# fuxiao0719/PanopticNeRF

Measured on AMD Instinct MI355X. Metric: Msamples/sec (coarse+fine), KITTI-360 1408x376, higher is better.
Workload: dtype bf16

## Files before the change

### panopticnerf_amd/csrc/asm/gen_mlp_tt.py

```python
#!/usr/bin/env python3
import struct
import sys
from contextlib import contextmanager

V_T2 = 15
NSLOT, SLOT = 4, 33 * 1024
P = 4
D, SKIP = 8, 4

V_TID, V_LANE16, V_FRAG, V_BIAS, V_T0, V_DMA, V_LB4, V_TRACE = 0, 1, 2, 6, 10, 11, 14, 15
V_T1 = 1
V_RING, V_ACC = 16, 32
V_EX, V_ED = 160, 192
V_G = 208
V_ZZ, V_ZN, V_DN, V_LW = 240, 242, 244, 246
V_IN = 224
V_TMP = 208
V_PTMP = 248
V_AUXA = V_PTMP + 6
V_LWA = V_IN + 2
A0, A1 = 0, 128
S_IMG, S_RAYS, S_Z, S_S, S_N, S_MAGIC, S_SHIFT, S_NGRP, S_NWG, S_REC, S_RECF, S_PS, S_NSEM, S_NINST, S_CLK = 4, 6, 8, 10, 11, 12, 13, 14, 15, 16, 18, 20, 22, 23, 24
S_WAVE, S_W4K, S_GRP, S_PIECE, S_T0, S_T1 = 26, 27, 28, 30, 34, 35
S_VALID, S_LAST = 36, 40
# ... 32 lines not shown
    def __init__(self, kind, base):
        self.kind, self.base = kind, base

    def reg(self, i, n=1):
        return (ar if self.kind == "a" else vr)(self.base + i, n)


class Sim:
    def __init__(self, name, cap):
        self.name, self.cap, self.q, self.n = name, cap, [], 0

    def push(self, certain=True):
        self.n += 1
        self.q.append((self.n, certain))
        return self.n

    def wait_count(self, tag):
        if tag is None or not any(t == tag for t, _ in self.q):
            return None
        idx = [t for t, _ in self.q].index(tag)
        n = sum(1 for _, c in self.q[idx + 1:] if c)
        n = min(n, self.cap)
        self.q = self.q[idx + 1:]
        return n

    def drain(self):
        self.q = []

    def state(self):
        return [c for _, c in self.q]


class Gen:
    def __init__(self, nbs, nbi, name, trace=False, abl=0, depth=2, softmax=False, tap=0):
        self.depth = depth
        self.tap = tap
        self.softmax = softmax
        self.nbs, self.nbi, self.name, self.trace, self.abl = nbs, nbi, name, trace, abl
        self.nstamp = 0
        self.o = []
        self.nlabel = 0
        self.lgkm = Sim("lgkm", 15)
        self.vm = Sim("vm", 63)
        self.side, self.side_lo, self.outbox, self.capture = [], [], [], None
        self.ring_tags = [None] * P
        self.piece_tag = {}
        self.pending_pack = None
        self.g2_acc = self.park_acc = None
        self.m0 = None
        self.logit_units = []
        self.acc_free = list(range(8))
        self.lwr_acc = self.lwr_tag = None
        self.aux_tags = {}
        self.build_plan()
        self.build_units()
        self.stream = []
        for u in self.units:
            u["frag0"] = len(self.stream)
            self.stream += [(sl, of) for sl, of, _, _ in self.unit_frags(u)]

    def build_plan(self):
        L = []

        def add(name, nblk, segs, fbc, mode):
            nks = sum(n for _, n in segs)
            if fbc * nks + 1 > 33:
                fbc = 1
            L.append(dict(name=name, nblk=nblk, segs=segs, nks=nks, fbc=fbc, mode=mode))
        for i in range(D):
            if i == 0:
                add("L0", 8, [("ex", 4)], 8, "relu")
            elif i - 1 == SKIP:
                add("L%d" % i, 8, [("ex", 4), ("h", 16)], 2, "relu")
            else:
                add("L%d" % i, 8, [("h", 16)], 2, "relu")
        add("feature", 8, [("h", 16)], 2, "linear")
        add("views", 4, [("F", 16), ("ed", 2)], 2, "relu")
        add("rgbs", 1, [("g", 8), ("hh", 16)], 1, "rgbs")
        if self.depth == 1:
            if self.nbs:
                add("sem1", self.nbs, [("tap", 16)], self.nbs, "logits")
            if self.nbi:
                add("inst1", 1, [("tap", 16)], 1, "logits")
        else:
            if self.nbs:
                add("sem0", 4, [("tap", 16)], 2, "relu")
            if self.nbi:
                add("inst0", 4, [("tap", 16)], 2, "relu")
            if self.nbs:
                add("sem1", self.nbs, [("shs", 8)], self.nbs, "logits")
            if self.nbi:
                add("inst1", 1, [("shi", 8)], 1, "logits")
# ... 494 lines not shown
            e("s_lshl_b32 s%d, s%d, 3" % (S_T0, S_GRP))
            e("s_lshl_b32 s%d, s%d, 1" % (S_SAVE, S_WAVE))
            e("s_add_u32 s%d, s%d, s%d" % (S_T0, S_T0, S_SAVE))
            e("s_add_u32 s%d, s%d, %d" % (S_T0, S_T0, t))
            e("s_mul_i32 s%d, s%d, s%d" % (S_SAVE, S_T0, S_RECF))
            e("s_mul_hi_i32 s%d, s%d, s%d" % (S_SAVE + 1, S_T0, S_RECF))
            e("s_lshl_b64 s[%d:%d], s[%d:%d], 2" % (S_SAVE, S_SAVE + 1, S_SAVE, S_SAVE + 1))
            e("s_add_u32 s%d, s%d, s%d" % (S_REC_T + 2 * t, S_REC, S_SAVE))
            e("s_addc_u32 s%d, s%d, s%d" % (S_REC_T + 2 * t + 1, S_REC + 1, S_SAVE + 1))
            e("s_lshl_b32 s%d, s%d, 2" % (S_SAVE, S_NSEM))
            e("s_add_u32 s%d, s%d, s%d" % (S_REC_I + 2 * t, S_REC_T + 2 * t, S_SAVE))
            e("s_addc_u32 s%d, s%d, 0" % (S_REC_I + 2 * t + 1, S_REC_T + 2 * t + 1))
            e("s_lshl_b32 s%d, s%d, 5" % (S_T0, S_T0))
            e("v_and_b32 v%d, 31, v%d" % (d, V_TID))
            e("v_or_b32 v%d, s%d, v%d" % (d, S_T0, d))
            e("v_lshlrev_b32 v%d, 4, v%d" % (d, d))
            e("v_mov_b32 v%d, v%d" % (T[4], V_LW + t))
            e("v_mov_b32 v%d, v%d" % (T[5], acc + 0))
            e("v_mov_b32 v%d, v%d" % (T[6], acc + 1))
            e("v_mov_b32 v%d, v%d" % (T[7], acc + 2))
            e("s_and_b64 s[%d:%d], s[%d:%d], s[%d:%d]" % (S_SAVE, S_SAVE + 1, VAL, VAL + 1, S_HI0, S_HI0 + 1))
            e("s_mov_b64 exec, s[%d:%d]" % (S_SAVE, S_SAVE + 1))
            self.vm_op("global_store_dwordx4 v%d, %s, s[%d:%d]" % (d, vr(T[4], 4), S_PS, S_PS + 1))
            e("s_mov_b64 exec, 1")
            e("v_mov_b32 v%d, s%d" % (x, S_Q))
            e("v_mov_b32 v%d, 0" % d)
            self.vm_op("global_store_dword v%d, v%d, s[%d:%d]" % (d, x, S_REC_T + 2 * t, S_REC_T + 2 * t + 1))
            e("s_mov_b64 exec, -1")
        self.q(28, stores)

    def acc_reg(self, i):
        return V_ACC + 16 * i

    def acc_take(self, n):
        assert len(self.acc_free) >= n, ("accumulators exhausted", self.acc_free)
        got, self.acc_free = self.acc_free[:n], self.acc_free[n:]
        return got

    def acc_release(self, ids):
        self.acc_free = sorted(set(self.acc_free) | set(ids))

    def arm_plan(self, u):
        c = self.chunks[u["chunk"]]
        l = self.layers[u["layer"]]
        slot = u["chunk"] % NSLOT
        bias_off = c["nfb"] * l["nks"] * 1024
        u["accs"], u["arm_tags"] = {}, []
        plans = []
        for bi, blk in enumerate(u["blocks"]):
            b_in_chunk = blk - c["fb"]
            for t in range(2):
                key = (bi, t)
                ops = []

                def take(key=key):
                    while not self.acc_free and self.side_busy():
                        self.drain_side(8)
                    u["accs"][key] = self.acc_take(1)[0]
                if t == 1:
                    plans.append([take])
                    continue
                if l["mode"] == "logits":
                    def first(key=key, slot=slot, take=take):
                        take()
                        self.e("v_add_u32 v%d, 0x%x, v%d" % (self.acc_reg(u["accs"][key]), slot * SLOT, V_LB4))
                    ops.append(first)
                    for r in list(range(1, 16)) + [0]:
                        ops.append(lambda key=key, r=r, off=bias_off + b_in_chunk * 128: u["arm_tags"].append(
                            self.lds_read("ds_read_b32 v%d, v%d offset:%d" % (self.acc_reg(u["accs"][key]) + r, self.acc_reg(u["accs"][key]), off))))
                else:
                    for m in range(4):
                        def rd(key=key, m=m, off=bias_off + b_in_chunk * 128 + m * 32, take=take):
                            if m == 0:
                                take()
                            a = self.acc_reg(u["accs"][key])
                            u["arm_tags"].append(self.lds_read("ds_read_b128 %s, v%d offset:%d" % (vr(a + 4 * m, 4), V_BIAS + slot, off)))
                        ops.append(rd)
                plans.append(ops)
        return plans

    def pack_ops(self, u):
        l = self.layers[u["layer"]]
        if not self.trace:
            return self.pack_ops_pipelined(u)
        out = []
        for bi, blk in enumerate(u["blocks"]):
            for t in range(2):
                a = self.acc_reg(u["accs"][(bi, t)])
                dst = self.out_block(l, blk, t)
                for p in range(8):
                    def fn(a=a, p=p, dst=dst, relu=(l["mode"] == "relu"), k=len(out)):
# ... 34 lines not shown
                self.e("v_pk_max_i16 v%d, v%d, 0" % (d if kind == "v" else T[k % 3], T[k % 3]))

        def store(k):
            _, kind, d, _ = pairs[k]
            if kind == "a":
                self.e("v_accvgpr_write_b32 a%d, v%d" % (d, T[k % 3]))

        def final_at(k):
            kind = pairs[k][1]
            return k + 2 if kind == "a" else (k + 1 if relu else k)
        out = []
        for j in range(n + 2):
            def fn(j=j):
                if 0 <= j - 2 < n:
                    store(j - 2)
                if 0 <= j - 1 < n:
                    activate(j - 1)
                if j < n:
                    convert(j)
            done = [(pairs[k][1], pairs[k][2]) for k in range(max(0, j - 2), min(n, j + 1)) if final_at(k) == j]
            out.append((done, fn, pairs[min(j, n - 1)][3]))
        return out

    @staticmethod
    def tile_at(ks, t):
        return 1 - t if ks == 0 else t

    def b_operand(self, u, ks, t):
        l = self.layers[u["layer"]]
        seg, k = self.seg_of_ks(l, ks)
        li = u["layer"]
        return self.loc_of(seg, li, t, k)

    def emit_unit(self, ui, side_budget=3):
        U = self.units
        u = U[ui]
        l = self.layers[u["layer"]]
        c = self.chunks[u["chunk"]]
        frags = self.unit_frags(u)
        nm = 2 * len(frags)
        swap = l["mode"] == "logits"
        e = self.e
        e("; ==== unit %d: %s blocks %s (chunk %d, slot %d), %d MFMAs" % (ui, l["name"], u["blocks"], u["chunk"], u["chunk"] % NSLOT, nm))
        self.stamp(ui)
        if l["name"] == "L%d" % (SKIP + 2) and u["blocks"][0] == 0:
            self.queue_inputs_early()
        if l["name"] == "views" and u["blocks"] == [0]:
            self.drain_side()
        if l["name"] == "views" and u["blocks"] == [1]:
            self.park()
        if l["name"] == (("sem0" if self.nbs else "inst0") if self.depth == 2 else "sem1") and u["blocks"][0] == 0:
            self.unpark()
        if l["name"] == "views" and u["blocks"] == [2]:
            self.g2_acc = self.acc_take(1)[0]
        prev = self.pending_pack
        self.pending_pack = None
        packs = prev["ops"] if prev else []
        reads = {}
        for i in range(nm):
            f, t = i // 2, i % 2
            loc = self.b_operand(u, frags[f][2], self.tile_at(frags[f][2], t))
            for r in range(4):
                reads.setdefault((loc.kind, loc.base + r), i)
        nxt = U[ui + 1] if ui + 1 < len(U) else None
        plans = self.arm_plan(nxt) if nxt is not None else []
        musts, dls, pack_fns = [], [], set()
        by_acc = {}
        for dst, fn, a in packs:
            by_acc.setdefault(a, []).append((dst, fn))
        k = 0
        for a, lst in by_acc.items():
            for dst, fn in lst:
                musts.append(fn if not self.abl & 4 else (lambda: None))
                pack_fns.add(musts[-1])
                if isinstance(dst, list):
                    dd = [reads[d] for d in dst if d in reads]
                    dls.append(min(dd) if dd else None)
                else:
                    dls.append(reads.get(dst))
            musts.append(lambda a=a: self.acc_release([a]))
            dls.append(None)
            if k < len(plans):
                for op in plans[k]:
                    musts.append(op)
                    dls.append(None)
                k += 1
        for kk in range(k, len(plans)):
            for op in plans[kk]:
                musts.append(op)
                dls.append(None)
        lwr_from = None
        if nxt is None and (self.logit_units or l["mode"] == "logits"):
            lwr_from = len(musts)
            for op in self.lwr_ops():
                musts.append(op)
                dls.append(None)
        n = len(musts)
        pos = []
        late = not packs and n > 0 and nxt is not None
        for j in range(n):
            spread = 1 + (j * max(1, nm - 6)) // max(1, n) if not late else (2 * nm) // 3 + (j * max(1, nm // 3 - 5)) // max(1, n)
            pos.append(spread if dls[j] is None else min(spread, max(0, dls[j] - 2)))
        if lwr_from is not None:
            nl = n - lwr_from
            for j in range(lwr_from, n):
                pos[j] = max(pos[j], min(nm - 2, nm // 2 + ((j - lwr_from) * max(1, nm // 2 - 3)) // nl))
        for j in range(n - 2, -1, -1):
            pos[j] = min(pos[j], pos[j + 1])
        must_at = {}
        for j, g in enumerate(pos):
            must_at.setdefault(g, []).append(j)
        piece_at = {}
        cu = [k for k, x in enumerate(U) if x["chunk"] == u["chunk"]]
        c3 = (u["chunk"] + 3) % self.NC
        npieces = self.pieces_of(c3)
        k_in = cu.index(ui)
        mine = [j for j in range(npieces) if (j * len(cu)) // npieces == k_in]
        cost = [3 * sum(1 for j in must_at.get(g, []) if j < n and dls[j] is not None or (j < n and musts[j] in pack_fns)) +
                sum(1 for j in must_at.get(g, [])) for g in range(nm)]
        for idx, j in enumerate(mine):
            span = max(len(mine) + 1, nm - 3)
            lo = 1 + (idx * span) // max(1, len(mine))
            hi = max(lo + 1, 1 + ((idx + 1) * span) // max(1, len(mine)))
            g = min(range(lo, min(hi, nm - 1)), key=lambda x: (cost[x], x))
            cost[g] += 2
            piece_at.setdefault(g, []).append(j)
        first_wait_done = False
        for i in range(nm):
            f, t = i // 2, i % 2
            slot, off, ks, bi = frags[f]
            gi = u["frag0"] + f
            if t == 0:
                if not first_wait_done:
                    for tg in u["arm_tags"][-1:]:
                        self.wait_lgkm(tg)
                    first_wait_done = True
                self.wait_lgkm(self.ring_tags[gi % P])
            tile = self.tile_at(ks, t)
            a = self.acc_reg(u["accs"][(bi, tile)])
            c_in = self.acc_reg(u["accs"][(bi, 0)]) if ks == 0 else a
            bloc = self.b_operand(u, ks, tile)
            ring = vr(V_RING + 4 * (gi % P), 4)
            if swap:
                e("v_mfma_f32_32x32x16_bf16 %s, %s, %s, %s" % (vr(a, 16), bloc.reg(0, 4), ring, vr(c_in, 16)))
            else:
                e("v_mfma_f32_32x32x16_bf16 %s, %s, %s, %s" % (vr(a, 16), ring, bloc.reg(0, 4), vr(c_in, 16)))
            if t == 1:
                gn = gi + P - 1
                if gn < len(self.stream):
                    sl, of = self.stream[gn]
                    self.ring_tags[gn % P] = self.lds_read("ds_read_b128 %s, v%d offset:%d" % (vr(V_RING + 4 * (gn % P), 4), V_FRAG + sl, of))
            for j in must_at.get(i, []):
                musts[j]()
            for j in ([] if self.abl & 1 else piece_at.get(i, [])):
                if j == 0:
                    self.chunk_base(c3)
                tg = self.piece(c3, j)
                self.piece_tag[c3] = tg
            self.drain_side(1 if l["name"].startswith("L") or l["name"] in ("feature", "views") else 3 if late else 2)
        for g in sorted(must_at):
            assert g < nm, (g, nm)
        if l["mode"] in ("relu", "linear"):
            self.pending_pack = dict(ops=self.pack_ops(u), accs=list(u["accs"].values()))
        elif l["mode"] == "rgbs":
            for t in range(2):
                self.rgbs_epilogue(t, self.acc_reg(u["accs"][(0, t)]))
            ids = list(u["accs"].values())
            self.q(0, lambda: self.defer(lambda: self.acc_release(ids)))
            self.queue_inputs_late()
            self.acc_release([self.g2_acc])
            self.g2_acc = None
            if not self.nbs:
                self.unpark()
        else:
            self.logit_units.append(u)
        if u["last_of_chunk"]:
            c2 = (u["chunk"] + 2) % self.NC
            if not self.abl & 2:
                self.wait_vm(self.piece_tag.get(c2))
                e("s_barrier")
            d = u["chunk"] + 1
            while d < self.NC and self.chunks[d].get("dummy"):
                e("; ==== dummy chunk %d (slot %d)" % (d, d % NSLOT))
                c3 = (d + 3) % self.NC
# ... 145 lines not shown
            for r in ([] if self.softmax else range(16)):
                for t in ts:
                    for k, (u, bi, blk, inst) in enumerate(blocks):
                        a = self.acc_reg(u["accs"][(bi, t)])
                        if r == 0:
                            e("v_fma_f32 v%d, v%d, v%d, 0" % (sums[t][k], lwr_reg(t, 0), a))
                        else:
                            e("v_fmac_f32 v%d, v%d, v%d" % (sums[t][k], lwr_reg(t, r), a + r))
            for t in ts:
                tags[t] = [self.lds_read("ds_bpermute_b32 v%d, v%d, v%d" % (oth[t][k], adr, sums[t][k])) for k in range(nb)]

        def stores(t):
            for k in range(nb):
                self.wait_lgkm(tags[t][k])
                e("v_add_f32 v%d, v%d, v%d" % (oth[t][k], sums[t][k], oth[t][k]))
            for k, (u, bi, blk, inst) in enumerate(blocks):
                e("s_mov_b64 exec, s[%d:%d]" % (S_MSK + 2 * k, S_MSK + 2 * k + 1))
                base = (S_REC_I if inst else S_REC_T) + 2 * t
                self.vm_op("global_store_dword v%d, v%d, s[%d:%d] offset:%d" % (V_LB4, oth[t][k], base, base + 1, 4 + 128 * blk))
            e("s_mov_b64 exec, -1")
        self.stamp(len(self.units) + 4)
        if self.softmax:
            self.tail_softmax(blocks, lwr_reg, tag_lwr)
        fmas((0, 1))
        self.stamp(len(self.units) + 5)
        stores(0)
        stores(1)
        for u in self.logit_units:
            self.acc_release(list(u["accs"].values()))
        self.acc_release(self.lwr_acc)
        self.lwr_acc = None
        self.logit_units = []

    def queue_inputs_early(self):
        def which():
            with self.atomic():
                self.e("s_add_u32 s%d, s%d, s%d" % (S_GRP2, S_GRP, S_NWG))
                self.e("s_cmp_lt_i32 s%d, s%d" % (S_GRP2, S_NGRP))
                self.e("s_cselect_b32 s%d, s%d, s%d" % (S_GRP2, S_GRP2, S_GRP))
        self.q(3, which)
        tags = {}
        for t in range(2):
            self.q(34, (lambda t=t: tags.__setitem__(t, self.fetch_tile(t, S_GRP2))))
        for t in range(2):
            self.q(1, (lambda t=t: self.wait_vm(tags[t])))
            for cost, fn in self.encode_tile(t, "x"):
                self.q(cost, fn)

    PARK = (3, 6, 7, 0)

    def park(self):
        self.park_acc = self.acc_take(1)[0]
        for t in range(2):
            for i, k in enumerate(Gen.PARK):
                self.e("v_mov_b32 v%d, v%d" % (self.acc_reg(self.park_acc) + len(Gen.PARK) * t + i, V_IN + 8 * t + k))

    def unpark(self):
        for t in range(2):
            for i, k in enumerate(Gen.PARK):
                self.e("v_mov_b32 v%d, v%d" % (V_IN + 8 * t + k, self.acc_reg(self.park_acc) + len(Gen.PARK) * t + i))
        self.acc_release([self.park_acc])
        self.park_acc = None

    def queue_inputs_late(self):
        for t in range(2):
            for cost, fn in self.encode_tile(t, "d"):
                self.q(cost, fn, low=True)

    def stamp(self, idx):
        if not self.trace:
            return
        pair = S_CLK0 + 2 * (self.nstamp & 1)
        prev = S_CLK0 + 2 * ((self.nstamp + 1) & 1)
        if self.last_stamp is not None:
            self.o.append("\tv_writelane_b32 v%d, s%d, %d" % (V_TRACE, prev, self.last_stamp))
        self.o.append("\ts_memtime s[%d:%d]" % (pair, pair + 1))
        self.last_stamp = idx
        self.nstamp += 1
        if idx == len(self.units) + 3:
            skip = self.label()
            self.o += ["\ts_waitcnt lgkmcnt(0)", "\ts_and_b32 s%d, s101, 7" % S_T0, "\ts_add_u32 s%d, s%d, 56" % (S_T0, S_T0),
                       "\ts_mov_b32 m0, s%d" % S_T0, "\ts_nop 1",
                       "\tv_writelane_b32 v%d, s%d, m0" % (V_TRACE, pair),
                       "\ts_and_b32 s%d, s101, 31" % S_T0, "\ts_cmp_eq_u32 s%d, 0" % S_T0, "\ts_cbranch_scc0 %s" % skip,
                       "\ts_lshr_b32 s%d, s101, 5" % S_T0, "\ts_add_u32 s%d, s%d, 48" % (S_T0, S_T0), "\ts_mov_b32 m0, s%d" % S_T0,
                       "\ts_nop 1", "\tv_writelane_b32 v%d, s%d, m0" % (V_TRACE, pair), skip + ":",
                       "\ts_add_u32 s101, s101, 1"]

    def prefetch_first_unit(self):
        u0 = self.units[0]
        for plan in self.arm_plan(u0):
            for op in plan:
                op()
        for g in range(P - 1):
            sl, of = self.stream[g]
            self.ring_tags[g % P] = self.lds_read("ds_read_b128 %s, v%d offset:%d" % (vr(V_RING + 4 * (g % P), 4), V_FRAG + sl, of))

    def advance_group_state(self):
        e = self.e
        for t in range(2):
            vi = V_IN + 8 * t
            e("v_mov_b32 v%d, v%d" % (V_ZZ + t, vi + 6))
            e("v_mov_b32 v%d, v%d" % (V_ZN + t, vi + 7))
            e("v_mov_b32 v%d, v%d" % (V_DN + t, vi + 0))
            e("s_mov_b64 s[%d:%d], s[%d:%d]" % (S_VALID + 2 * t, S_VALID + 2 * t + 1, S_NVALID + 2 * t, S_NVALID + 2 * t + 1))
            e("s_mov_b64 s[%d:%d], s[%d:%d]" % (S_LAST + 2 * t, S_LAST + 2 * t + 1, S_NLAST + 2 * t, S_NLAST + 2 * t + 1))

    def group_body(self):
        self.m0 = None
        assert self.acc_free == [i for i in range(8) if i not in self.units[0]["accs"].values()], self.acc_free
        self.last_stamp = None
        for ui in range(len(self.units)):
# ... 58 lines not shown
                    e("v_and_b32 v%d, 31, v0" % V_T0)
                    if nblk > 1:
                        e("v_add_u32 v%d, %d, v%d" % (V_T0, 32 * (nblk - 1), V_T0))
                    e("v_cmp_gt_i32 s[%d:%d], s%d, v%d" % (S_VMSK + 2 * k, S_VMSK + 2 * k + 1, sreg, V_T0))
        lend, lloop, lfin = self.label(), self.label(), self.label()
        e("s_mov_b32 s%d, s2" % S_GRP)
        e("s_cmp_ge_i32 s%d, s%d" % (S_GRP, S_NGRP))
        e("s_cbranch_scc1 %s" % lend)
        for c in range(3):
            self.chunk_base(c)
            for j in range(self.pieces_of(c)):
                self.piece_tag[c] = self.piece(c, j)
        e("s_waitcnt vmcnt(0)")
        self.vm.drain()
        e("s_barrier")
        e("s_mov_b32 s%d, s%d" % (S_GRP2, S_GRP))
        tags = [self.fetch_tile(t, S_GRP2) for t in range(2)]
        for t in range(2):
            self.wait_vm(tags[t])
            for part in ("x", "d"):
                for _, fn in self.encode_tile(t, part):
                    fn()
        self.advance_group_state()
        if not self.trace:
            e("s_memtime s[%d:%d]" % (S_CLK0, S_CLK0 + 1))
            e("s_memrealtime s[%d:%d]" % (S_CLK0 + 2, S_CLK0 + 3))
        else:
            e("v_mov_b32 v%d, 0" % V_TRACE)
            e("s_mov_b32 s101, 0")
            e("s_memtime s[90:91]")
            e("s_waitcnt lgkmcnt(0)")
        e("s_waitcnt lgkmcnt(0)")
        self.lgkm.drain()
        self.prefetch_first_unit()
        keep = self.o
        self.o = []
        self.group_body()
        self.prefetch_first_unit()
        self.o = keep
        self.o.append(lloop + ":")
        self.group_body()
        e("s_add_u32 s%d, s%d, s%d" % (S_GRP, S_GRP, S_NWG))
        e("s_cmp_ge_i32 s%d, s%d" % (S_GRP, S_NGRP))
        e("s_cbranch_scc1 %s" % lend)
        self.prefetch_first_unit()
        e("s_branch %s" % lloop)
        self.o.append(lend + ":")
        e("s_waitcnt vmcnt(0) lgkmcnt(0)")
        e("s_cmp_eq_u64 s[%d:%d], 0" % (S_CLK, S_CLK + 1))
        e("s_cbranch_scc1 %s" % lfin)
        if self.trace:
            lw = self.label()
            e("s_cmp_lg_u32 s%d, 0" % S_WAVE)
            e("s_cbranch_scc1 %s" % lw)
            e("s_memtime s[%d:%d]" % (S_CLK0, S_CLK0 + 1))
            e("s_waitcnt lgkmcnt(0)")
            e("s_sub_u32 s%d, s%d, s90" % (S_CLK0, S_CLK0))
            e("s_lshl_b32 s%d, s2, 2" % S_T0)
            e("s_add_u32 s%d, s%d, 256" % (S_T0, S_T0))
            e("v_mov_b32 v%d, s%d" % (V_T0, S_T0))
            e("v_mov_b32 v%d, s%d" % (V_T1, S_CLK0))
            e("s_mov_b64 exec, 1")
            e("global_store_dword v%d, v%d, s[%d:%d]" % (V_T0, V_T1, S_CLK, S_CLK + 1))
            e("s_mov_b64 exec, -1")
            e("s_waitcnt vmcnt(0)")
            self.o.append(lw + ":")
        e("s_cmp_lg_u32 s2, 0")
        e("s_cbranch_scc1 %s" % lfin)
        if self.trace:
            e("s_cmp_lg_u32 s%d, 0" % S_WAVE)
            e("s_cbranch_scc1 %s" % lfin)
            e("v_and_b32 v%d, 63, v0" % V_T0)
            e("v_lshlrev_b32 v%d, 2, v%d" % (V_T0, V_T0))
            e("global_store_dword v%d, v%d, s[%d:%d]" % (V_T0, V_TRACE, S_CLK, S_CLK + 1))
            e("s_waitcnt vmcnt(0)")
            e("s_branch %s" % lfin)
        e("s_memtime s[%d:%d]" % (S_T0 - 0, S_T0 + 1))
        e("s_memrealtime s[%d:%d]" % (S_SAVE, S_SAVE + 1))
        e("s_waitcnt lgkmcnt(0)")
        e("s_sub_u32 s%d, s%d, s%d" % (S_T0, S_T0, S_CLK0))
        e("s_subb_u32 s%d, s%d, s%d" % (S_T1, S_T1, S_CLK0 + 1))
        e("s_sub_u32 s%d, s%d, s%d" % (S_SAVE, S_SAVE, S_CLK0 + 2))
        e("s_subb_u32 s%d, s%d, s%d" % (S_SAVE + 1, S_SAVE + 1, S_CLK0 + 3))
        e("v_cmp_eq_u32 vcc, 0, v0")
        e("s_and_saveexec_b64 s[%d:%d], vcc" % (S_VALID, S_VALID + 1))
        e("s_cbranch_execz %s" % lfin)
        e("v_mov_b32 v20, s%d" % S_T0)
        e("v_mov_b32 v21, s%d" % S_T1)
        e("v_mov_b32 v22, s%d" % S_SAVE)
        e("v_mov_b32 v23, s%d" % (S_SAVE + 1))
        e("v_mov_b32 v%d, 0" % V_T0)
        e("global_store_dwordx4 v%d, v[20:23], s[%d:%d]" % (V_T0, S_CLK, S_CLK + 1))
        e("s_waitcnt vmcnt(0)")
        self.o.append(lfin + ":")
        e("s_endpgm")
        self.o += [".Lend_%s:" % name, "\t.size\t%s, .Lend_%s-%s" % (name, name, name), ""]
        self.o += ["\t.rodata", "\t.p2align\t6", "\t.amdhsa_kernel %s" % name,
                   "\t\t.amdhsa_group_segment_fixed_size %d" % (NSLOT * SLOT + 1024),
                   "\t\t.amdhsa_private_segment_fixed_size 0", "\t\t.amdhsa_kernarg_size %d" % KERNARG_BYTES, "\t\t.amdhsa_user_sgpr_count 2",
                   "\t\t.amdhsa_user_sgpr_kernarg_segment_ptr 1", "\t\t.amdhsa_system_sgpr_workgroup_id_x 1",
                   "\t\t.amdhsa_system_vgpr_workitem_id 0", "\t\t.amdhsa_next_free_vgpr 512", "\t\t.amdhsa_next_free_sgpr 102",
                   "\t\t.amdhsa_accum_offset 256", "\t\t.amdhsa_reserve_vcc 1", "\t\t.amdhsa_float_denorm_mode_32 3",
                   "\t\t.amdhsa_float_denorm_mode_16_64 3", "\t\t.amdhsa_dx10_clamp 1", "\t\t.amdhsa_ieee_mode 1",
                   "\t.end_amdhsa_kernel", ""]
        return "\n".join(self.o)


KERNARG_BYTES = 104


def metadata(names):
    o = ["\t.amdgpu_metadata", "---", "amdhsa.kernels:"]
    for n in names:
        o += ["  - .agpr_count:     256", "    .args:", "      - .offset:         0", "        .size:           %d" % KERNARG_BYTES,
              "        .value_kind:     by_value", "    .group_segment_fixed_size: %d" % (NSLOT * SLOT + 1024),
              "    .kernarg_segment_align: 8", "    .kernarg_segment_size: %d" % KERNARG_BYTES, "    .max_flat_workgroup_size: 256",
              "    .name:           %s" % n, "    .private_segment_fixed_size: 0", "    .sgpr_count:     108",
              "    .sgpr_spill_count: 0", "    .symbol:         %s.kd" % n, "    .uniform_work_group_size: 1",
              "    .uses_dynamic_stack: false", "    .vgpr_count:     512", "    .vgpr_spill_count: 0", "    .wavefront_size: 64"]
    o += ["amdhsa.target:   amdgcn-amd-amdhsa--gfx950", "amdhsa.version:", "  - 1", "  - 2", "...", "\t.end_amdgpu_metadata", ""]
    return "\n".join(o)


def variant_name(tap, depth, sm, nbs, nbi):
    tag = ("f" if tap else "") + ("d1" if depth == 1 else "") + ("sm" if sm else "")
    return "k_mlp_tt_%ss%di%d" % (tag + "_" if tag else "", nbs, nbi)


def main():
    out = sys.argv[1] if len(sys.argv) > 1 else "/dev/stdout"
    parts = ['\t.amdgcn_target "amdgcn-amd-amdhsa--gfx950"', "\t.amdhsa_code_object_version 5", ""]
    names = []
    for nbs, nbi in ((1, 1), (2, 1), (0, 0), (1, 0), (2, 0), (3, 0)):
        n = "k_mlp_tt_s%di%d" % (nbs, nbi)
        names.append(n)
        parts.append(Gen(nbs, nbi, n).kernel())
    for tap in (0, 1):
        for depth in (2, 1):
# ... 26 lines not shown
```

### panopticnerf_amd/csrc/pnr_mlp.hip

```cpp
#include <stdlib.h>
#include <string.h>

#include "pnr_mlp_plan.h"

int pnr_mlp_validate(const pnr_mlp_desc* d);

#include "pnr_mlp_core.h"
#include "pnr_mlp_pp.h"
#include "pnr_mlp_fuse.h"
#include "pnr_mlp_tt.h"
#define PNR_QUERY_MAX_POINTS (((int64_t)1 << 31) - 4096)
template <int PREC, int TILES, class CTX, int KIND, int NA, int NB, int NFB_OUT, int MODE, int NOUT>
__device__ __forceinline__ void layer_regs(CTX& c, const uint32_t (&inA)[TILES][NA],
                                           const uint32_t (&inB)[TILES][NB > 0 ? NB : 1],
                                           uint32_t (&out)[TILES][NOUT], uint16_t* save = nullptr,
                                           const int* srow = nullptr)
{
    constexpr int RPB = PrecT<PREC>::RPB;
    constexpr int KS = NA / 4 + NB / 4;
    constexpr int FBC0 = pnr_layer_fbc(KIND, PREC);
    constexpr int FBC = (NFB_OUT % FBC0 == 0) ? FBC0 : 1;
    constexpr int G = (CTX::GDB / FBC) < 1 ? 1 : (CTX::GDB / FBC);
    static_assert(NOUT >= NFB_OUT * RPB, "output register array too small");
#pragma unroll
// ... 814 lines not shown
{
    int rc = pnr_mlp_validate(desc);
    if (rc != PNR_OK) return rc;
    PNR_REQUIRE(desc->precision == PNR_PREC_BF16, "pnr_mlp_forward_composite: bf16 only");
    PNR_REQUIRE(desc->plan != 4, "pnr_mlp_forward_composite: a plan-4 (field) image is for pnr_mlp_query only");
    PNR_REQUIRE(n_rays >= 1 && n_samples >= 32 && n_samples <= 256 && (n_samples & 31) == 0,
                "pnr_mlp_forward_composite: n_samples=%d must be a multiple of 32 in [32,256]", n_samples);
    PNR_REQUIRE(desc->n_sem + desc->n_inst <= 128, "pnr_mlp_forward_composite: n_sem + n_inst <= 128");
    PNR_REQUIRE(packed && rays && z && workspace, "pnr_mlp_forward_composite: null pointer");
    PNR_REQUIRE(n_rays * (int64_t)n_samples < ((int64_t)1 << 31) - 4096, "pnr_mlp_forward_composite: R*N exceeds 2^31");
    PNR_REQUIRE((((uintptr_t)rays | (uintptr_t)packed | (uintptr_t)workspace) & 15) == 0,
                "pnr_mlp_forward_composite: rays / packed / workspace must be 16-byte aligned");
    PnrPlan plan;
    pnr_build_plan(*desc, plan);
    mlp_args_fill(a, desc, plan, packed);
    a.rays = rays; a.z = z; a.S = (int)(n_rays * n_samples); a.N = n_samples;
    pnr_set_div_magic(n_samples, a.n_magic, a.n_shift);
    a.rec_floats = record_floats(*desc);
    a.rec = (float*)workspace;
    const int64_t tiles = ((int64_t)a.S + 255) / 256 * 8;
    a.ps = (float4*)(a.rec + tiles * a.rec_floats);
    hipStream_t st = (hipStream_t)stream;
    const bool softmax = (desc->flags & PNR_MLP_SOFTMAX) && desc->n_sem + desc->n_inst > 0;
    if (desc->plan == 3)
        return desc->W == 256 ? launch_mlp_pp<256, false, true, 0, true>(a, st) : launch_mlp_pp<128, false, true, 0, true>(a, st);
    if (desc->plan == 2) {
        PnrTTArgs t;
        memset(&t, 0, sizeof(t));
        t.image = a.data; t.rays = rays; t.z = z; t.S = a.S; t.N = a.N; t.n_magic = a.n_magic; t.n_shift = a.n_shift;
        t.rec = a.rec; t.rec_floats = a.rec_floats; t.ps = a.ps; t.n_sem = a.n_sem; t.n_inst = a.n_inst; t.clk = a.clk;
        PNR_REQUIRE(n_rays < ((int64_t)1 << 24), "pnr_mlp_forward_composite: the two-tile kernel addresses 2^24 rays per launch");
        uint32_t* aux = (uint32_t*)(((uintptr_t)((uint8_t*)a.ps + (int64_t)a.S * 16 + 256) + PNR_RAY_AUX_BYTES - 1)
                                    & ~(uintptr_t)(PNR_RAY_AUX_BYTES - 1));
        k_ray_aux<<<dim3((unsigned)((2 * n_rays + 255) / 256)), dim3(256), 0, st>>>(rays, n_rays, aux);
        t.aux = aux;
        t.n_wg = (desc->flags >> 16) & 0x1FF;
        const bool trace = (desc->flags & 0xFF00) == PNR_MLP_TRACE;
        return pnr_mlp_tt_launch(t, (desc->n_sem + 31) / 32, (desc->n_inst + 31) / 32, a.head_depth, a.head_tap, softmax, st, trace,
                                 trace ? ((desc->flags >> 4) & 7) : 0);
    }
    if (desc->plan == 1) {
        const int nbs = (desc->n_sem + 31) / 32, nbi = (desc->n_inst + 31) / 32;
        switch (4 * nbs + nbi + (softmax ? 16 : 0)) {
        case 4: return launch_mlp_pp<256, false, true, 4>(a, st);
        case 5: return launch_mlp_pp<256, false, true, 5>(a, st);
        case 8: return launch_mlp_pp<256, false, true, 8>(a, st);
        case 9: return launch_mlp_pp<256, false, true, 9>(a, st);
        case 20: return launch_mlp_pp<256, false, true, 20>(a, st);
        case 21: return launch_mlp_pp<256, false, true, 21>(a, st);
        case 24: return launch_mlp_pp<256, false, true, 24>(a, st);
        case 25: return launch_mlp_pp<256, false, true, 25>(a, st);
        default: PNR_REQUIRE(false, "pnr_mlp_forward_composite: no plan-1 kernel for %d + %d logit blocks", nbs, nbi);
        }
    }
    PNR_REQUIRE(!softmax, "pnr_mlp_forward_composite: softmax compositing needs the plan-1 image (pnr_mlp_fused_plan >= 1, desc.plan = 1)");
    return desc->W == 256 ? launch_mlp_pp<256, false, true>(a, st) : launch_mlp_pp<128, false, true>(a, st);
}

PNR_EXPORT int pnr_mlp_forward_tiles(const pnr_mlp_desc* desc, const void* packed, const float* rays, const float* z, int64_t n_rays,
                                     int n_samples, void* workspace, void* stream)
{
    PNR_REQUIRE(n_rays >= 0, "pnr_mlp_forward_tiles: bad size");
    if (n_rays == 0) return PNR_OK;
    MlpArgs a;
    return fused_mlp_launch(desc, packed, rays, z, n_rays, n_samples, workspace, stream, a);
}

PNR_EXPORT int pnr_composite_combine(const pnr_mlp_desc* desc, const void* workspace, const float* z, int64_t n_rays, int n_samples,
                                     const int32_t* label_sem, const int32_t* label_inst, int white_bkgd, float* rgb, float* depth,
                                     float* acc, float* weights, float* sem, float* inst, float* fix_sem, float* fix_inst, void* stream)
{
    int rc = pnr_mlp_validate(desc);
// ... 234 lines not shown
```

### panopticnerf_amd/csrc/pnr_mlp_tt.cpp

```cpp
#include <mutex>
#include <string>

#include "pnr_common.h"
#include "pnr_mlp_tt.h"

static const unsigned char k_co[] = {
#include "pnr_mlp_tt_co.inc"
};

namespace {
struct DevTable {
    hipModule_t mod = nullptr;
    hipFunction_t fn[8][4][2] = {};
    hipFunction_t fn_trace[8] = {};
    bool tried = false, ok = false;
};
DevTable g_tab[64];
std::mutex g_mu;
}

static int tt_table(DevTable*& out, int capturing = 0)
{
    int dev = 0;
    PNR_HIP(hipGetDevice(&dev));
// ... 20 lines not shown
            if (a) snprintf(nm, sizeof(nm), "k_mlp_tt_s2i1_trace_a%d", a); else snprintf(nm, sizeof(nm), "k_mlp_tt_s2i1_trace");
            if (hipModuleGetFunction(&t.fn_trace[a], t.mod, nm) != hipSuccess) { t.fn_trace[a] = nullptr; (void)hipGetLastError(); }
        }
        if (e != hipSuccess) {
            pnr_set_error("pnr_mlp_tt: loading the two-tile code object failed: %s (the first call on a device must not be inside a "
                          "stream capture)", hipGetErrorString(e));
            if (loaded) (void)hipModuleUnload(t.mod);
            t = DevTable();
            (void)hipGetLastError();
            return PNR_EHIP;
        }
        t.ok = true;
    }
    PNR_REQUIRE(t.ok, "pnr_mlp_tt: the two-tile code object is not loaded");
    out = &t;
    return PNR_OK;
}

int pnr_mlp_tt_prepare(void)
{
    DevTable* t = nullptr;
    return tt_table(t);
}

void pnr_mlp_tt_prepare_quiet(void)
{
    int n = 0;
    if (hipGetDeviceCount(&n) != hipSuccess || n <= 0) { (void)hipGetLastError(); return; }
    const std::string keep = pnr_last_error();
    DevTable* t = nullptr;
    if (tt_table(t) != PNR_OK) pnr_set_error("%s", keep.c_str());
}

int pnr_mlp_tt_launch(const PnrTTArgs& a, int nbs, int nbi, int head_depth, int head_tap, bool softmax, hipStream_t stream, bool trace, int trace_abl)
{
    PNR_REQUIRE(nbs >= 0 && nbs <= 3 && nbi >= 0 && nbi <= (nbs == 1 || nbs == 2 ? 1 : 0), "pnr_mlp_forward_composite: no two-tile kernel for %d + %d logit blocks", nbs, nbi);
    PNR_REQUIRE(a.S >= 1 && a.S < (1 << 28), "pnr_mlp_forward_composite: the two-tile kernel takes R*N < 2^28 samples per launch (got %d): "
                "render in chunks", a.S);
    DevTable* t = nullptr;
    hipStreamCaptureStatus cs = hipStreamCaptureStatusNone;
    PNR_HIP(hipStreamIsCapturing(stream, &cs));
    int rc = tt_table(t, cs != hipStreamCaptureStatusNone);
    if (rc != PNR_OK) return rc;
    hipFunction_t fn = t->fn[!nbs ? 0 : (head_tap ? 4 : 0) + (softmax ? 2 : 0) + (head_depth == 1 ? 1 : 0)][nbs][nbi];
    PNR_REQUIRE(fn, "pnr_mlp_tt: no kernel for %d + %d logit blocks at head_depth %d", nbs, nbi, head_depth);
    if (trace) {
        PNR_REQUIRE(head_depth != 1 && !softmax && !head_tap, "pnr_mlp_tt: the trace build exists for head_depth 2, head_tap 0, logits compositing");
        PNR_REQUIRE(nbs == 2 && nbi == 1 && a.clk, "pnr_mlp_tt: the trace build exists for 2 + 1 logit blocks and needs the clock buffer");
        fn = t->fn_trace[trace_abl & 7];
        PNR_REQUIRE(fn, "pnr_mlp_tt: PNR_MLP_TRACE%s%d is not in this library: the trace kernels are diagnostics builds "
                    "(make EXTRA_TT=trace, ablations EXTRA_TT=abl)", trace_abl & 7 ? " ablation " : " ", trace_abl & 7);
    }
    PnrTTArgs ka = a;
    const int cus = pnr_cu_count();
    ka.n_groups = (a.S + 255) / 256;
    const int cap = (a.n_wg > 0 && a.n_wg < cus) ? a.n_wg : cus;
    ka.n_wg = ka.n_groups < cap ? ka.n_groups : cap;
    size_t size = sizeof(ka);
    void* extra[] = {HIP_LAUNCH_PARAM_BUFFER_POINTER, &ka, HIP_LAUNCH_PARAM_BUFFER_SIZE, &size, HIP_LAUNCH_PARAM_END};
    PNR_HIP(hipModuleLaunchKernel(fn, (unsigned)ka.n_wg, 1, 1, 256, 1, 1, 0, stream, nullptr, extra));
    return PNR_OK;
}
```

### panopticnerf_amd/csrc/pnr_mlp_tt.h

```cpp
#pragma once
#include <hip/hip_runtime.h>
#include <stdint.h>

struct PnrTTArgs {
    const void* image;
    const float* rays;
    const float* z;
    int32_t S, N;
    uint32_t n_magic;
    int32_t n_shift;
    int32_t n_groups, n_wg;
    float* rec;
    int32_t rec_floats, pad0;
    void* ps;
    int32_t n_sem, n_inst;
    unsigned long long* clk;
    const void* aux;
    uint64_t reserved;
};
static_assert(sizeof(PnrTTArgs) == 104, "k_mlp_tt reads its arguments at fixed offsets");

int pnr_mlp_tt_prepare(void);
void pnr_mlp_tt_prepare_quiet(void);
int pnr_mlp_tt_launch(const PnrTTArgs& a, int nbs, int nbi, int head_depth, int head_tap, bool softmax, hipStream_t stream, bool trace = false,
                      int trace_abl = 0);
```

Measured before the change: 1188.

## Rotate group loop so logit reduction and stores overlap next group's first unit

The assembly generator gains a rotated loop schedule for kernels with semantic logits and no softmax. The final logit-unit reduction (FMA chain, lane exchange via ds_bpermute, global stores) and the bias arming for the next group are moved into filler slots inside the first unit of the next trip, and the fragment ring prefetch wraps across the group boundary. This is meant to hide the epilogue behind the next group's MFMAs. A dry-run search picks accumulator assignments that repeat from trip to trip, which adds generator complexity and register-allocation risk. On the host side, kernel resolution and validation now run before the ray-aux launch, so a failed lookup no longer leaves an orphan launch.

```diff
diff --git a/panopticnerf_amd/csrc/asm/gen_mlp_tt.py b/panopticnerf_amd/csrc/asm/gen_mlp_tt.py
--- a/panopticnerf_amd/csrc/asm/gen_mlp_tt.py
+++ b/panopticnerf_amd/csrc/asm/gen_mlp_tt.py
@@ -88,7 +88,11 @@
 
 
 class Gen:
-    def __init__(self, nbs, nbi, name, trace=False, abl=0, depth=2, softmax=False, tap=0):
+    def __init__(self, nbs, nbi, name, trace=False, abl=0, depth=2, softmax=False, tap=0, forced=None):
+        self.args = dict(nbs=nbs, nbi=nbi, name=name, trace=trace, abl=abl, depth=depth, softmax=softmax, tap=tap)
+        self.rotate = bool(nbs) and not softmax
+        self.forced = forced
+        self.flip = None
         self.depth = depth
         self.tap = tap
         self.softmax = softmax
@@ -114,6 +118,21 @@
         for u in self.units:
             u["frag0"] = len(self.stream)
             self.stream += [(sl, of) for sl, of, _, _ in self.unit_frags(u)]
+        if self.rotate:
+            self.rot_setup()
+
+    def rot_setup(self):
+        U = self.units
+        lu = [i for i, u in enumerate(U) if self.layers[u["layer"]]["mode"] == "logits"]
+        last = len(U) - 1
+        assert lu and lu == list(range(lu[0], last + 1)), lu
+        self.nm_last = 2 * len(self.unit_frags(U[last]))
+        self.early = len(lu) >= 2
+        self.lwr_unit = last - 1 if (self.early and self.nm_last < 32) else last
+        self.tight = U[last]["chunk"] == self.NC - 1
+        self.wrap_ring = self.tight and len(self.stream) % P == 0
+        self.arm_in_last = self.tight and self.early
+        assert 2 * len(self.unit_frags(U[0])) == 16 and len(U[0]["blocks"]) == 2
 
     def build_plan(self):
         L = []
@@ -674,9 +693,12 @@
     def acc_reg(self, i):
         return V_ACC + 16 * i
 
-    def acc_take(self, n):
+    def acc_take(self, n, high=False):
         assert len(self.acc_free) >= n, ("accumulators exhausted", self.acc_free)
-        got, self.acc_free = self.acc_free[:n], self.acc_free[n:]
+        if high:
+            got, self.acc_free = self.acc_free[-n:], self.acc_free[:-n]
+        else:
+            got, self.acc_free = self.acc_free[:n], self.acc_free[n:]
         return got
 
     def acc_release(self, ids):
@@ -698,7 +720,7 @@
                 def take(key=key):
                     while not self.acc_free and self.side_busy():
                         self.drain_side(8)
-                    u["accs"][key] = self.acc_take(1)[0]
+                    u["accs"][key] = self.acc_take(1, high=self.flip is not None and u is self.units[self.flip])[0]
                 if t == 1:
                     plans.append([take])
                     continue
@@ -799,7 +821,7 @@
         li = u["layer"]
         return self.loc_of(seg, li, t, k)
 
-    def emit_unit(self, ui, side_budget=3):
+    def emit_unit(self, ui, side_budget=3, fillers=None):
         U = self.units
         u = U[ui]
         l = self.layers[u["layer"]]
@@ -809,7 +831,7 @@
         swap = l["mode"] == "logits"
         e = self.e
         e("; ==== unit %d: %s blocks %s (chunk %d, slot %d), %d MFMAs" % (ui, l["name"], u["blocks"], u["chunk"], u["chunk"] % NSLOT, nm))
-        self.stamp(ui)
+        self.stamp(ui if fillers is None else len(U) + 1)
         if l["name"] == "L%d" % (SKIP + 2) and u["blocks"][0] == 0:
             self.queue_inputs_early()
         if l["name"] == "views" and u["blocks"] == [0]:
@@ -857,7 +879,7 @@
                 musts.append(op)
                 dls.append(None)
         lwr_from = None
-        if nxt is None and (self.logit_units or l["mode"] == "logits"):
+        if ui == self.lwr_unit if self.rotate else (nxt is None and (self.logit_units or l["mode"] == "logits")):
             lwr_from = len(musts)
             for op in self.lwr_ops():
                 musts.append(op)
@@ -868,7 +890,14 @@
         for j in range(n):
             spread = 1 + (j * max(1, nm - 6)) // max(1, n) if not late else (2 * nm) // 3 + (j * max(1, nm // 3 - 5)) // max(1, n)
             pos.append(spread if dls[j] is None else min(spread, max(0, dls[j] - 2)))
-        if lwr_from is not None:
+        lwr_g0 = max(1, nm // 2 - 10)
+        if lwr_from is not None and self.rotate and self.early:
+            for j in range(lwr_from, n):
+                if nxt is None:
+                    pos[j] = lwr_g0 + (j - lwr_from) // 2
+                else:
+                    pos[j] = max(pos[j], nm - 2 - (n - 1 - j) // 2)
+        elif lwr_from is not None:
             nl = n - lwr_from
             for j in range(lwr_from, n):
                 pos[j] = max(pos[j], min(nm - 2, nm // 2 + ((j - lwr_from) * max(1, nm // 2 - 3)) // nl))
@@ -892,6 +921,9 @@
             g = min(range(lo, min(hi, nm - 1)), key=lambda x: (cost[x], x))
             cost[g] += 2
             piece_at.setdefault(g, []).append(j)
+        extra_at = dict(fillers) if fillers is not None else {}
+        if self.rotate and nxt is None:
+            extra_at = self.rot_last_plan(nm, lwr_g0 + 10 if self.lwr_unit == ui else 1)
         first_wait_done = False
         for i in range(nm):
             f, t = i // 2, i % 2
@@ -914,9 +946,13 @@
                 e("v_mfma_f32_32x32x16_bf16 %s, %s, %s, %s" % (vr(a, 16), ring, bloc.reg(0, 4), vr(c_in, 16)))
             if t == 1:
                 gn = gi + P - 1
+                if gn >= len(self.stream) and self.rotate and self.wrap_ring:
+                    gn -= len(self.stream)
                 if gn < len(self.stream):
                     sl, of = self.stream[gn]
                     self.ring_tags[gn % P] = self.lds_read("ds_read_b128 %s, v%d offset:%d" % (vr(V_RING + 4 * (gn % P), 4), V_FRAG + sl, of))
+            for fn in extra_at.get(i, []):
+                fn()
             for j in must_at.get(i, []):
                 musts[j]()
             for j in ([] if self.abl & 1 else piece_at.get(i, [])):
@@ -1128,6 +1164,144 @@
         self.lwr_acc = None
         self.logit_units = []
 
+    def rot_blocks(self):
+        return [(u, bi, blk, self.layers[u["layer"]]["name"] == "inst1") for u in self.logit_units for bi, blk in enumerate(u["blocks"])]
+
+    @staticmethod
+    def rot_regs(k, t):
+        return ((V_PTMP + k, V_PTMP + 3 + k), (V_IN + 1 + k, (V_IN + 4, V_IN + 5, V_IN + 9)[k]))[t]
+
+    def rot_chain(self, blocks, k0):
+        def lwr_reg(t, r):
+            return self.acc_reg(self.lwr_acc[t]) + 4 * (r >> 2) + (((r & 3) + 2) & 3)
+        ops = []
+        for r in range(16):
+            for t in range(2):
+                for k, (u, bi, blk, inst) in enumerate(blocks):
+                    def fma(r=r, t=t, k=k0 + k, u=u, bi=bi):
+                        a = self.acc_reg(u["accs"][(bi, t)])
+                        if r == 0:
+                            self.e("v_fma_f32 v%d, v%d, v%d, 0" % (self.rot_regs(k, t)[0], lwr_reg(t, 0), a))
+                        else:
+                            self.e("v_fmac_f32 v%d, v%d, v%d" % (self.rot_regs(k, t)[0], lwr_reg(t, r), a + r))
+                    ops.append(fma)
+        return ops
+
+    def rot_arm_ops(self):
+        return [op for plan in self.arm_plan(self.units[0]) for op in plan]
+
+    def rot_last_plan(self, nm, g0):
+        at = {}
+        early = self.rot_blocks()
+        if not early:
+            return at
+        g1 = nm - 4 if self.arm_in_last else nm - 2
+        assert g0 + 4 <= g1, (g0, g1)
+
+        def start():
+            self.drain_side()
+            self.stamp(0)
+            self.wait_lgkm(self.lwr_tag)
+        ops = [start] + self.rot_chain(early, 0)
+        for i, fn in enumerate(ops):
+            at.setdefault(g0 + (i * (g1 - g0 + 1)) // len(ops), []).append(fn)
+        at[g1].append(lambda: self.acc_release([a for u in self.logit_units for a in u["accs"].values()]))
+        if self.arm_in_last:
+            for i, fn in enumerate(self.rot_arm_ops()):
+                at.setdefault(g1 + 1 + i // 4, []).append(fn)
+            at.setdefault(nm - 2, []).append(self.advance_group_state)
+        return at
+
+    def rot_boundary(self):
+        nu = len(self.units)
+        blocks = self.rot_blocks()
+        last = [b for b in blocks if b[0] is self.logit_units[-1]]
+        k0 = len(blocks) - len(last)
+        chain = self.rot_chain(last, k0)
+        held = list(self.logit_units[-1]["accs"].values())
+
+        def release():
+            self.acc_release(held + self.lwr_acc)
+            self.lwr_acc = None
+            self.logit_units = []
+            self.stamp(nu + 2)
+        if not self.early:
+            self.stamp(0)
+        if not self.arm_in_last:
+            if len(self.acc_free) < 4:
+                self.wait_lgkm(self.lwr_tag)
+                for fn in chain:
+                    fn()
+                chain = []
+                release()
+            for fn in self.rot_arm_ops():
+                fn()
+            self.advance_group_state()
+        if not self.wrap_ring:
+            for g in range(P - 1):
+                sl, of = self.stream[g]
+                self.ring_tags[g % P] = self.lds_read("ds_read_b128 %s, v%d offset:%d" % (vr(V_RING + 4 * (g % P), 4), V_FRAG + sl, of))
+        at = {}
+        adr = V_PTMP + 7
+        tags = {}
+
+        def setup():
+            self.e("v_xor_b32 v%d, 32, v%d" % (adr, V_TID))
+            self.e("v_and_b32 v%d, 63, v%d" % (adr, adr))
+            self.e("v_lshlrev_b32 v%d, 2, v%d" % (adr, adr))
+            if chain:
+                self.wait_lgkm(self.lwr_tag)
+        at[0] = [setup]
+        for i, fn in enumerate(chain):
+            at.setdefault(i // 4, []).append(fn)
+        gb = 0
+        if chain:
+            gb = (len(chain) - 1) // 4 + 1
+            at[gb - 1].append(release)
+
+        def exchange():
+            for t in range(2):
+                for k in range(len(blocks)):
+                    s, o = self.rot_regs(k, t)
+                    tags[(t, k)] = self.lds_read("ds_bpermute_b32 v%d, v%d, v%d" % (o, adr, s))
+        at.setdefault(gb, []).append(exchange)
+
+        def stores(t):
+            for k in range(len(blocks)):
+                s, o = self.rot_regs(k, t)
+                self.wait_lgkm(tags[(t, k)])
+                self.e("v_add_f32 v%d, v%d, v%d" % (o, s, o))
+            for k, (u, bi, blk, inst) in enumerate(blocks):
+                self.e("s_mov_b64 exec, s[%d:%d]" % (S_MSK + 2 * k, S_MSK + 2 * k + 1))
+                base = (S_REC_I if inst else S_REC_T) + 2 * t
+                self.vm_op("global_store_dword v%d, v%d, s[%d:%d] offset:%d" % (V_LB4, self.rot_regs(k, t)[1], base, base + 1, 4 + 128 * blk))
+            self.e("s_mov_b64 exec, -1")
+        at.setdefault(gb + 3, []).append(lambda: stores(0))
+        at.setdefault(gb + 4, []).append(lambda: (stores(1), self.stamp(nu + 3)))
+        assert max(at) < 16, sorted(at)
+        return at
+
+    def group_body_rot(self):
+        self.m0 = None
+        self.last_stamp = None
+        nu = len(self.units)
+        for ui in range(1, nu):
+            self.emit_unit(ui)
+        self.stamp(nu)
+        self.drain_side()
+        fillers = self.rot_boundary()
+        self.emit_unit(0, fillers=fillers)
+        assert self.lwr_acc is None and not self.logit_units
+        self.stamp(nu + 4)
+
+    def loop_sig(self):
+        u0, u1 = self.units[0], self.units[1]
+        ring = sorted(h.v for h in self.ring_tags if h is not None)[-(P - 1):]
+        live = ring + [u1["arm_tags"][-1].v]
+        lg = [(self.lgkm.n - t, c) for t, c in self.lgkm.q if t >= min(live)]
+        return dict(accs=(dict(u0["accs"]), dict(u1["accs"]), list(self.acc_free)), lg=(lg, [self.lgkm.n - v for v in live]),
+                    vm=self.vm.state())
+
     def queue_inputs_early(self):
         def which():
             with self.atomic():
@@ -1169,11 +1343,14 @@
         pair = S_CLK0 + 2 * (self.nstamp & 1)
         prev = S_CLK0 + 2 * ((self.nstamp + 1) & 1)
         if self.last_stamp is not None:
+            if len(self.o) - self.stamp_at < 24:
+                self.o.append("\ts_waitcnt lgkmcnt(0)")
             self.o.append("\tv_writelane_b32 v%d, s%d, %d" % (V_TRACE, prev, self.last_stamp))
         self.o.append("\ts_memtime s[%d:%d]" % (pair, pair + 1))
+        self.stamp_at = len(self.o)
         self.last_stamp = idx
         self.nstamp += 1
-        if idx == len(self.units) + 3:
+        if idx == len(self.units) + (4 if self.rotate else 3):
             skip = self.label()
             self.o += ["\ts_waitcnt lgkmcnt(0)", "\ts_and_b32 s%d, s101, 7" % S_T0, "\ts_add_u32 s%d, s%d, 56" % (S_T0, S_T0),
                        "\ts_mov_b32 m0, s%d" % S_T0, "\ts_nop 1",
@@ -1298,6 +1475,55 @@
             e("s_waitcnt lgkmcnt(0)")
         e("s_waitcnt lgkmcnt(0)")
         self.lgkm.drain()
+        if self.rotate:
+            self.rotated_loop(lloop)
+        else:
+            self.plain_loop(lend, lloop)
+        self.kernel_end(lend, lfin)
+        return "\n".join(self.o)
+
+    def rotated_loop(self, lloop):
+        e = self.e
+        if self.forced is None:
+            for flip in [None] + [i for i, u in enumerate(self.units) if len(u["blocks"]) == 1 and i + 1 < len(self.units)]:
+                dry = Gen(forced="learn", **self.args)
+                dry.flip = flip
+                dry.kernel()
+                if dry.learned is not None:
+                    break
+            else:
+                raise AssertionError("no accumulator assignment that repeats from trip to trip")
+            self.forced, self.flip = dry.learned, flip
+        if self.forced != "learn":
+            u0, u1, _ = self.forced
+            order = [u[k] for u in (u0, u1) for k in ((0, 0), (0, 1), (1, 0), (1, 1))]
+            self.acc_free = order + [a for a in range(8) if a not in order]
+        self.prefetch_first_unit()
+        self.last_stamp = None
+        self.emit_unit(0)
+        entry = self.loop_sig()
+        keep = self.o
+        self.o = []
+        sigs = []
+        for _ in range(3 if self.forced == "learn" else 1):
+            self.group_body_rot()
+            sigs.append(self.loop_sig())
+        self.o = keep
+        if self.forced == "learn":
+            self.learned = sigs[-1]["accs"] if sigs[-1] == sigs[-2] else None
+            return
+        self.o.append(lloop + ":")
+        self.group_body_rot()
+        sigs.append(self.loop_sig())
+        assert sigs[0] == sigs[1], ("the trip's end state is not its start state", sigs)
+        assert entry["accs"] == sigs[1]["accs"] and entry["lg"] == sigs[1]["lg"], (entry, sigs[1])
+        assert sigs[1]["vm"][len(sigs[1]["vm"]) - len(entry["vm"]):] == entry["vm"], (entry["vm"], sigs[1]["vm"])
+        e("s_add_u32 s%d, s%d, s%d" % (S_GRP, S_GRP, S_NWG))
+        e("s_cmp_lt_i32 s%d, s%d" % (S_GRP, S_NGRP))
+        e("s_cbranch_scc1 %s" % lloop)
+
+    def plain_loop(self, lend, lloop):
+        e = self.e
         self.prefetch_first_unit()
         keep = self.o
         self.o = []
@@ -1311,6 +1537,9 @@
         e("s_cbranch_scc1 %s" % lend)
         self.prefetch_first_unit()
         e("s_branch %s" % lloop)
+
+    def kernel_end(self, lend, lfin):
+        e, name = self.e, self.name
         self.o.append(lend + ":")
         e("s_waitcnt vmcnt(0) lgkmcnt(0)")
         e("s_cmp_eq_u64 s[%d:%d], 0" % (S_CLK, S_CLK + 1))
@@ -1369,7 +1598,6 @@
                    "\t\t.amdhsa_accum_offset 256", "\t\t.amdhsa_reserve_vcc 1", "\t\t.amdhsa_float_denorm_mode_32 3",
                    "\t\t.amdhsa_float_denorm_mode_16_64 3", "\t\t.amdhsa_dx10_clamp 1", "\t\t.amdhsa_ieee_mode 1",
                    "\t.end_amdhsa_kernel", ""]
-        return "\n".join(self.o)
 
 
 KERNARG_BYTES = 104
diff --git a/panopticnerf_amd/csrc/pnr_mlp.hip b/panopticnerf_amd/csrc/pnr_mlp.hip
--- a/panopticnerf_amd/csrc/pnr_mlp.hip
+++ b/panopticnerf_amd/csrc/pnr_mlp.hip
@@ -870,12 +870,16 @@
         PNR_REQUIRE(n_rays < ((int64_t)1 << 24), "pnr_mlp_forward_composite: the two-tile kernel addresses 2^24 rays per launch");
         uint32_t* aux = (uint32_t*)(((uintptr_t)((uint8_t*)a.ps + (int64_t)a.S * 16 + 256) + PNR_RAY_AUX_BYTES - 1)
                                     & ~(uintptr_t)(PNR_RAY_AUX_BYTES - 1));
-        k_ray_aux<<<dim3((unsigned)((2 * n_rays + 255) / 256)), dim3(256), 0, st>>>(rays, n_rays, aux);
         t.aux = aux;
         t.n_wg = (desc->flags >> 16) & 0x1FF;
         const bool trace = (desc->flags & 0xFF00) == PNR_MLP_TRACE;
-        return pnr_mlp_tt_launch(t, (desc->n_sem + 31) / 32, (desc->n_inst + 31) / 32, a.head_depth, a.head_tap, softmax, st, trace,
-                                 trace ? ((desc->flags >> 4) & 7) : 0);
+        hipFunction_t fn = nullptr;
+        rc = pnr_mlp_tt_resolve(t.S, t.clk != nullptr, (desc->n_sem + 31) / 32, (desc->n_inst + 31) / 32, a.head_depth, a.head_tap, softmax, st,
+                                trace, trace ? ((desc->flags >> 4) & 7) : 0, &fn);
+        if (rc != PNR_OK) return rc;
+        k_ray_aux<<<dim3((unsigned)((2 * n_rays + 255) / 256)), dim3(256), 0, st>>>(rays, n_rays, aux);
+        PNR_CHECK_LAUNCH("k_ray_aux");
+        return pnr_mlp_tt_launch(t, fn, st);
     }
     if (desc->plan == 1) {
         const int nbs = (desc->n_sem + 31) / 32, nbi = (desc->n_inst + 31) / 32;
diff --git a/panopticnerf_amd/csrc/pnr_mlp_tt.cpp b/panopticnerf_amd/csrc/pnr_mlp_tt.cpp
--- a/panopticnerf_amd/csrc/pnr_mlp_tt.cpp
+++ b/panopticnerf_amd/csrc/pnr_mlp_tt.cpp
@@ -76,11 +76,12 @@
     if (tt_table(t) != PNR_OK) pnr_set_error("%s", keep.c_str());
 }
 
-int pnr_mlp_tt_launch(const PnrTTArgs& a, int nbs, int nbi, int head_depth, int head_tap, bool softmax, hipStream_t stream, bool trace, int trace_abl)
+int pnr_mlp_tt_resolve(int S, bool have_clk, int nbs, int nbi, int head_depth, int head_tap, bool softmax, hipStream_t stream, bool trace,
+                       int trace_abl, hipFunction_t* out)
 {
     PNR_REQUIRE(nbs >= 0 && nbs <= 3 && nbi >= 0 && nbi <= (nbs == 1 || nbs == 2 ? 1 : 0), "pnr_mlp_forward_composite: no two-tile kernel for %d + %d logit blocks", nbs, nbi);
-    PNR_REQUIRE(a.S >= 1 && a.S < (1 << 28), "pnr_mlp_forward_composite: the two-tile kernel takes R*N < 2^28 samples per launch (got %d): "
-                "render in chunks", a.S);
+    PNR_REQUIRE(S >= 1 && S < (1 << 28), "pnr_mlp_forward_composite: the two-tile kernel takes R*N < 2^28 samples per launch (got %d): "
+                "render in chunks", S);
     DevTable* t = nullptr;
     hipStreamCaptureStatus cs = hipStreamCaptureStatusNone;
     PNR_HIP(hipStreamIsCapturing(stream, &cs));
@@ -90,11 +91,17 @@
     PNR_REQUIRE(fn, "pnr_mlp_tt: no kernel for %d + %d logit blocks at head_depth %d", nbs, nbi, head_depth);
     if (trace) {
         PNR_REQUIRE(head_depth != 1 && !softmax && !head_tap, "pnr_mlp_tt: the trace build exists for head_depth 2, head_tap 0, logits compositing");
-        PNR_REQUIRE(nbs == 2 && nbi == 1 && a.clk, "pnr_mlp_tt: the trace build exists for 2 + 1 logit blocks and needs the clock buffer");
+        PNR_REQUIRE(nbs == 2 && nbi == 1 && have_clk, "pnr_mlp_tt: the trace build exists for 2 + 1 logit blocks and needs the clock buffer");
         fn = t->fn_trace[trace_abl & 7];
         PNR_REQUIRE(fn, "pnr_mlp_tt: PNR_MLP_TRACE%s%d is not in this library: the trace kernels are diagnostics builds "
                     "(make EXTRA_TT=trace, ablations EXTRA_TT=abl)", trace_abl & 7 ? " ablation " : " ", trace_abl & 7);
     }
+    *out = fn;
+    return PNR_OK;
+}
+
+int pnr_mlp_tt_launch(const PnrTTArgs& a, hipFunction_t fn, hipStream_t stream)
+{
     PnrTTArgs ka = a;
     const int cus = pnr_cu_count();
     ka.n_groups = (a.S + 255) / 256;
diff --git a/panopticnerf_amd/csrc/pnr_mlp_tt.h b/panopticnerf_amd/csrc/pnr_mlp_tt.h
--- a/panopticnerf_amd/csrc/pnr_mlp_tt.h
+++ b/panopticnerf_amd/csrc/pnr_mlp_tt.h
@@ -22,5 +22,6 @@
 
 int pnr_mlp_tt_prepare(void);
 void pnr_mlp_tt_prepare_quiet(void);
-int pnr_mlp_tt_launch(const PnrTTArgs& a, int nbs, int nbi, int head_depth, int head_tap, bool softmax, hipStream_t stream, bool trace = false,
-                      int trace_abl = 0);
+int pnr_mlp_tt_resolve(int S, bool have_clk, int nbs, int nbi, int head_depth, int head_tap, bool softmax, hipStream_t stream, bool trace,
+                       int trace_abl, hipFunction_t* out);
+int pnr_mlp_tt_launch(const PnrTTArgs& a, hipFunction_t fn, hipStream_t stream);
```

New measurement: 1190 (median of 6 runs). About the same (+0.2%).
